# MycroftAI/mycroft-precise

Hardware: AMD Instinct MI355X
Metric: MFCC+GRU windows/sec (node); max concurrent real-time 16 kHz streams (higher is better)
Workload: dtype f32

## Files before the change

### include/precise_engine.h

```cpp
#ifndef PRECISE_ENGINE_H
#define PRECISE_ENGINE_H

#include <stddef.h>
#include <stdint.h>

#ifdef __cplusplus
extern "C" {
#endif

#define PE_ABI_VERSION 8

typedef enum pe_status {
    PE_OK = 0,
    PE_ERR_INVALID = 1,
    PE_ERR_HIP = 2,
    PE_ERR_UNSUPPORTED = 3,
    PE_ERR_NOMEM = 4,
    PE_ERR_EOF = 5
} pe_status;

typedef struct pe_params {
    int32_t sample_rate;
    int32_t window_samples;
    int32_t hop_samples;
// ... 65 lines not shown
                      float* feats_out_host);
int pe_update_vectors_device(pe_engine* e, const int16_t* pcm_dev, int32_t chunk_samples,
                             float* feats_out_dev, void* hip_stream);

int pe_get_vectors(pe_engine* e, float* feats_out_host);

int pe_set_vectors(pe_engine* e, const float* feats_host);

int pe_run_device(pe_engine* e, float* raw_out_dev, void* hip_stream);

int pe_predict(pe_engine* e, const float* feats_host, int32_t n, float* out_host);
int pe_predict_device(pe_engine* e, const float* feats_dev, int32_t n, float* out_dev,
                      void* hip_stream);

int pe_vectorize_raw(pe_engine* e, const double* audio_host, int64_t n_samples,
                     double* feats_out_host, int64_t max_frames, int64_t* n_frames_out);

int pe_vectorize_mels(pe_engine* e, const double* audio_host, int64_t n_samples,
                      double* mels_out_host, int64_t max_frames, int64_t* n_frames_out);

int pe_evaluate(pe_engine* e, const double* audio_host, int64_t n_samples, int32_t hop_frames,
                float* out_host, int64_t max_windows, int64_t* n_windows_out);

int pe_set_decoder(pe_engine* e, const double* cd, int32_t cd_len, int32_t min_out, int32_t out_range, double center);
int pe_set_trigger(pe_engine* e, int32_t chunk_size_bytes, double sensitivity, int32_t trigger_level);
int pe_set_decoder_model(pe_engine* e, int32_t model, const double* cd, int32_t cd_len, int32_t min_out, int32_t out_range, double center);
int pe_set_trigger_model(pe_engine* e, int32_t model, int32_t chunk_size_bytes, double sensitivity, int32_t trigger_level);
int pe_decode_device(pe_engine* e, const float* raw_dev, double* conf_out_dev, unsigned char* fired_out_dev, void* hip_stream);
int pe_decode(pe_engine* e, const float* raw_host, double* conf_out_host, unsigned char* fired_out_host);

typedef struct pe_info {
    int32_t n_streams, n_features, n_mfcc, units, n_layers, ring_slots, carry_capacity;
    int32_t mfcc_precision, gru_precision;
    int64_t device_bytes;
} pe_info;
int pe_get_info(const pe_engine* e, pe_info* out);

int pe_get_stream_state(pe_engine* e, int32_t* q_out, uint32_t* computed_out, uint32_t* emitted_out);

int pe_set_renumber_at(pe_engine* e, uint32_t call_number);

int pe_set_fused(pe_engine* e, int32_t enabled);

int pe_set_input_projection(pe_engine* e, int32_t enabled);

int pe_set_gru_waves(pe_engine* e, int32_t waves_per_tile);

int pe_set_gru_tiling(pe_engine* e, int32_t tiling);
int pe_get_gru_tiling(const pe_engine* e);

int pe_set_timing(pe_engine* e, int32_t enabled);
int pe_get_last_timing(pe_engine* e, float* mfcc_ms, float* gru_ms);

#ifdef __cplusplus
}
#endif
#endif
```

### mycroft_precise_amd/_lib.py

```python
import ctypes as C
import importlib.util
import os
import weakref

import numpy as np

HERE = os.path.dirname(os.path.abspath(__file__))
LIB_PATH = os.environ.get('PE_LIB') or os.path.join(HERE, 'libprecise_engine.so')

PE_OK, PE_ERR_INVALID, PE_ERR_HIP, PE_ERR_UNSUPPORTED, PE_ERR_NOMEM, PE_ERR_EOF = range(6)
ABI_VERSION = 8


class PeParams(C.Structure):
    _fields_ = [(n, C.c_int32) for n in (
        'sample_rate', 'window_samples', 'hop_samples', 'n_fft', 'n_filt', 'n_mfcc', 'n_features',
        'use_delta', 'mfcc_precision', 'gru_precision', 'vectorizer', 'ring_precision')]


class PeGruLayer(C.Structure):
    _fields_ = [('n_in', C.c_int32), ('units', C.c_int32),
                ('kernel', C.POINTER(C.c_float)), ('recurrent_kernel', C.POINTER(C.c_float)),
                ('bias', C.POINTER(C.c_float))]


class PeWeights(C.Structure):
    _fields_ = [('n_layers', C.c_int32), ('layers', C.POINTER(PeGruLayer)),
                ('dense_kernel', C.POINTER(C.c_float)), ('dense_bias', C.c_float)]


class PeInfo(C.Structure):
    _fields_ = [(n, C.c_int32) for n in (
        'n_streams', 'n_features', 'n_mfcc', 'units', 'n_layers', 'ring_slots', 'carry_capacity',
        'mfcc_precision', 'gru_precision')] + [('device_bytes', C.c_int64)]


EXPORTS = {
    'pe_abi_version': (C.c_int, []),
    'pe_last_global_error': (C.c_char_p, []),
    'pe_create': (C.c_int, [C.POINTER(PeParams), C.POINTER(C.c_double), C.POINTER(PeWeights), C.c_int32,
                            C.c_int32, C.POINTER(C.c_void_p)]),
    'pe_create_models': (C.c_int, [C.POINTER(PeParams), C.POINTER(C.c_double), C.POINTER(PeWeights), C.c_int32, C.c_int32,
                                   C.c_int32, C.POINTER(C.c_void_p)]),
    'pe_get_n_models': (C.c_int, [C.c_void_p]),
    'pe_destroy': (C.c_int, [C.c_void_p]),
    'pe_last_error': (C.c_char_p, [C.c_void_p]),
    'pe_clear': (C.c_int, [C.c_void_p, C.c_void_p]),
    'pe_update': (C.c_int, [C.c_void_p, C.c_void_p, C.c_int32, C.c_void_p]),
    'pe_update_device': (C.c_int, [C.c_void_p, C.c_void_p, C.c_int32, C.c_void_p, C.c_void_p]),
    'pe_update_device_keep': (C.c_int, [C.c_void_p, C.c_void_p, C.c_int32, C.c_void_p, C.c_void_p]),
    'pe_update_subset': (C.c_int, [C.c_void_p, C.c_void_p, C.c_int32, C.c_void_p, C.c_int32, C.c_void_p]),
    'pe_update_subset_device': (C.c_int, [C.c_void_p, C.c_void_p, C.c_int32, C.c_void_p, C.c_int32, C.c_void_p, C.c_void_p]),
    'pe_set_renumber_at': (C.c_int, [C.c_void_p, C.c_uint32]),
    'pe_host_alloc': (C.c_int, [C.c_void_p, C.c_size_t, C.POINTER(C.c_void_p)]),
    'pe_host_free': (C.c_int, [C.c_void_p, C.c_void_p]),
    'pe_update_async': (C.c_int, [C.c_void_p, C.c_void_p, C.c_int32, C.c_void_p]),
    'pe_wait': (C.c_int, [C.c_void_p]),
    'pe_reserve_updates': (C.c_int, [C.c_void_p, C.c_int32, C.c_int32]),
    'pe_update_many': (C.c_int, [C.c_void_p, C.c_void_p, C.c_int32, C.c_int32, C.c_void_p]),
    'pe_update_many_device': (C.c_int, [C.c_void_p, C.c_void_p, C.c_int32, C.c_int32, C.c_void_p, C.c_void_p]),
    'pe_update_vectors': (C.c_int, [C.c_void_p, C.c_void_p, C.c_int32, C.c_void_p]),
    'pe_update_vectors_device': (C.c_int, [C.c_void_p, C.c_void_p, C.c_int32, C.c_void_p, C.c_void_p]),
    'pe_get_vectors': (C.c_int, [C.c_void_p, C.c_void_p]),
    'pe_set_vectors': (C.c_int, [C.c_void_p, C.c_void_p]),
    'pe_run_device': (C.c_int, [C.c_void_p, C.c_void_p, C.c_void_p]),
    'pe_predict': (C.c_int, [C.c_void_p, C.c_void_p, C.c_int32, C.c_void_p]),
    'pe_predict_device': (C.c_int, [C.c_void_p, C.c_void_p, C.c_int32, C.c_void_p, C.c_void_p]),
# ... 391 lines not shown
```

### mycroft_precise_amd/csrc/engine.hip

```cpp
#include "../../include/precise_engine.h"
#include "pe_common.h"
#include "gru_cw_pack.h"
#include "mfcc_general_device.h"

#include <algorithm>
#include <cmath>
#include <cstdarg>
#include <cstdio>
#include <cstdlib>
#include <cstring>
#include <string>
#include <vector>

using namespace pe;

namespace {

thread_local std::string g_global_error;

struct DeviceBuf {
    void* p = nullptr;
    size_t bytes = 0;
};

// ... 1 lines not shown
    float dense_bias = 0.f;
    float* wxd = nullptr; float* wx = nullptr; float* wr1 = nullptr; float* wr2 = nullptr; float* bias = nullptr; float* wd = nullptr;
    float* cw_blob = nullptr;
    float* wide_buf[2][6] = {{nullptr}}; float* wide_wd = nullptr;
    float* wide3_buf[2][6] = {{nullptr}}; float* wide3_wd = nullptr;
    uint16_t* wx_bf16 = nullptr; uint16_t* wr_bf16 = nullptr; float* wd_bf16 = nullptr;
    uint32_t* b20_blob = nullptr;
    uint32_t* x3_blob = nullptr;
};
struct DecState {
    double* cd = nullptr; int cd_len = 0, min_out = 0, out_range = 0; double center = 0.5;
    double threshold = 0.5; int level = 3, rearm = -8; bool on = false;
};

}

struct pe_engine {
    pe_params prm{};
    int device = 0;
    int n_streams = 0, n_tiles = 0, n_padded = 0;
    int units = 0, n_in = 0, n_layers = 0;
    int ring_slots = 0;
    int mel_nnz = 0;
    std::string err;
    std::vector<void*> allocs;
    int64_t device_bytes = 0;
    StreamRec* rec = nullptr;
    int16_t* carry = nullptr;
    const int16_t* kept = nullptr; int kept_chunk = 0;
    const int16_t* call_head = nullptr; int call_head_chunk = 0; bool call_keep = false;
    uint32_t call_no = 1;
    uint32_t renumber_at = 0x7fff0000u;
    bool fused = true;
    int gru_waves = 0;
    bool general = false;
    int row_floats = kRowFloats;
    int carry_cap = kCarryCap;
    GeneralTables gtab{};
    int gru_tiling = -1;
    int n_cus = 256;
    float* ring = nullptr;
    float* proj_ring = nullptr;
    bool proj_ok = false, proj_on = false;
    std::vector<float> proj_w_host, proj_b_host;
    int max_updates = 1;
    uint32_t* ke_hist = nullptr;
    unsigned char* table_blob = nullptr;
    pe_wave::Layout table_layout{};
    int n_models = 1;
    std::vector<NetPack> nets;
    std::vector<DecState> dec;
    bool wide = false;
    int wide_kx4[2] = {1, 1};
    int32_t* activation = nullptr;
    DeviceBuf st_pcm, st_out, st_feats, st_mask, st_audio, st_mfcc, st_conf, st_fired, st_ids;
    std::vector<uint8_t> seen_ids;
    bool timing = false;
    hipEvent_t ev[3] = {nullptr, nullptr, nullptr};
    bool ev_valid = false, ev_has_gru = false;
    static constexpr int kAsyncDepth = 3;
    struct AsyncSlot {
        float* pin_out = nullptr; size_t pin_out_bytes = 0;
        DeviceBuf dev_in, dev_out;
        hipEvent_t copied = nullptr, done = nullptr;
        float* user_out = nullptr; size_t out_bytes = 0;
        bool direct_out = false, busy = false;
// ... 745 lines not shown
    e->user_dirty = true;
}

int check_chunk(pe_engine* e, const void* pcm, int chunk) {
    if (!e) return PE_ERR_INVALID;
    if (chunk == 0) return fail(e, PE_ERR_EOF, "empty chunk");
    if (chunk < 0 || !pcm) return fail(e, PE_ERR_INVALID, "bad pcm buffer / chunk_samples=%d", chunk);
    return PE_OK;
}

int flush_kept(pe_engine* e, hipStream_t s) {
    if (!e->kept) return PE_OK;
    PE_HIP(e, launch_materialize_carry(state_of(e, e->call_no + 1u), e->kept, e->kept_chunk, e->n_streams, s));
    e->kept = nullptr; e->kept_chunk = 0;
    return PE_OK;
}

bool keep_eligible(const pe_engine* e, const int16_t* pcm_dev, int chunk) {
    return !e->general && (chunk & 1) == 0 && (reinterpret_cast<uintptr_t>(pcm_dev) & 3u) == 0 && chunk >= frame_len_of(e->prm) - 1
        && chunk >= e->carry_cap - 1;
}

bool can_fuse(const pe_engine* e, int chunk) {
    if (!(e->fused && !e->general && !e->wide && e->table_layout.mel_pad == 10 && chunk <= emit_window(e->prm) - frame_len_of(e->prm))) return false;
    if (gru_args(e).x3) return false;
    if (e->prm.gru_precision == 0 && gru_small_regs(e->units) >= 6 && gru_args(e).waves_per_tile != 4) return false;
    if (e->prm.use_delta && e->prm.gru_precision == 0) {
        const GruArgs g = gru_args(e);
        if (g.cw && (g.waves_per_tile != 4 || e->ring_slots != kCwSlots || e->prm.n_features > kCwSlots)) return false;
    }
    return true;
}

int do_update(pe_engine* e, const int16_t* pcm_dev, int chunk, float* raw_out_dev, float* feats_out_dev,
              hipStream_t s, const int32_t* ids = nullptr, int n_active = 0, bool keep = false) {
    int rc;
    const bool t = e->timing;
    const bool keep_call = keep && !ids && keep_eligible(e, pcm_dev, chunk);
    if (keep_call && e->kept) {
        const char* a0 = reinterpret_cast<const char*>(e->kept);
        const char* a1 = a0 + (size_t)e->n_streams * e->kept_chunk * sizeof(int16_t);
        const char* b0 = reinterpret_cast<const char*>(pcm_dev);
        const char* b1 = b0 + (size_t)e->n_streams * chunk * sizeof(int16_t);
        if (b0 < a1 && a0 < b1)
            return fail(e, PE_ERR_INVALID, "pe_update_device_keep: this call's chunks overlap the previous call's (%p), which still hold the "
                        "streams' leftover samples -- alternate between at least two buffers, or use pe_update_device", (const void*)e->kept);
    }
    if (!keep_call && (rc = flush_kept(e, s))) return rc;
    e->call_head = keep_call ? e->kept : nullptr; e->call_head_chunk = e->kept_chunk; e->call_keep = keep_call;
    struct Reset { pe_engine* e; ~Reset() { e->call_head = nullptr; e->call_head_chunk = 0; e->call_keep = false; } } reset{e};
    e->kept = keep_call ? pcm_dev : nullptr; e->kept_chunk = keep_call ? chunk : 0;
    uint32_t call = 0;
    if ((rc = begin_state_call(e, s, &call))) return rc;
    if (t) { PE_HIP(e, hipEventRecord(e->ev[0], s)); }
    if (raw_out_dev && can_fuse(e, chunk)) {
        GruArgs g = gru_args(e);
        g.call = call;
        g.predict_ke = 1;
        g.chunk = chunk;
        g.out = raw_out_dev;
        if (ids) { g.ids = ids; g.n_streams = n_active; }
        const ModelSet ms = model_set(e, g);
        const ModelSet* const models = e->n_models > 1 ? &ms : nullptr;
        if (e->prm.mfcc_precision == 0) PE_HIP(e, launch_fused(mfcc_args<double>(e, pcm_dev, chunk, call, ids, n_active), tables<double>(e), g, e->n_cus, s, models, e->n_models));
        else PE_HIP(e, launch_fused(mfcc_args<float>(e, pcm_dev, chunk, call, ids, n_active), tables<float>(e), g, e->n_cus, s, models, e->n_models));
        if (t) { PE_HIP(e, hipEventRecord(e->ev[1], s)); PE_HIP(e, hipEventRecord(e->ev[2], s)); e->ev_valid = true; e->ev_has_gru = false; }
    } else {
        if ((rc = launch_mfcc(e, pcm_dev, chunk, s, call, ids, n_active))) return rc;
        if (t) { PE_HIP(e, hipEventRecord(e->ev[1], s)); }
        if (raw_out_dev) {
            if ((rc = launch_gru_ring(e, raw_out_dev, s, ids, n_active))) return rc;
        }
        if (t) { PE_HIP(e, hipEventRecord(e->ev[2], s)); e->ev_valid = true; e->ev_has_gru = raw_out_dev != nullptr; }
    }
    if (feats_out_dev) {
        GatherArgs g{e->n_streams, e->prm.n_features, e->prm.n_mfcc, e->ring_slots, e->prm.ring_precision, e->ring, state_of(e, e->call_no + 1u), feats_out_dev, e->row_floats};
        PE_HIP(e, launch_gather(g, s));
    }
    return PE_OK;
}

}

extern "C" {

int pe_abi_version(void) { return PE_ABI_VERSION; }
const char* pe_last_global_error(void) { return g_global_error.c_str(); }
const char* pe_last_error(const pe_engine* e) { return e ? e->err.c_str() : g_global_error.c_str(); }

namespace {
int create_engine(const pe_params* p, const double* mel_filters, const pe_weights* w, int32_t n_models, int32_t n_streams,
                  int32_t device, pe_engine** out) {
    if (!p || !mel_filters || !w || !out) return fail(nullptr, PE_ERR_INVALID, "null argument to pe_create");
    *out = nullptr;
    if (n_streams <= 0) return fail(nullptr, PE_ERR_INVALID, "n_streams must be positive, got %d", n_streams);
    if (p->n_fft < 16 || p->n_fft > kGeneralMaxFft || (!general_is_pow2(p->n_fft) && p->n_fft > kGeneralMaxBlueFft))
        return fail(nullptr, PE_ERR_UNSUPPORTED, "n_fft must be any length in 16..%d or a power of two up to %d (got %d)", kGeneralMaxBlueFft, kGeneralMaxFft, p->n_fft);
    if (p->n_mfcc < 1 || p->n_mfcc > kGeneralMaxMfcc) return fail(nullptr, PE_ERR_UNSUPPORTED, "n_mfcc must be in 1..%d (got %d)", kGeneralMaxMfcc, p->n_mfcc);
// ... 771 lines not shown
        }
        return PE_OK;
    }
    g.waves_per_tile = 1;
    return launch_networks_many(e, g, n_updates, s);
}

int pe_update_many(pe_engine* e, const int16_t* pcm_host, int32_t chunk, int32_t n_updates, float* raw_out_host) {
    int rc = check_chunk(e, pcm_host, chunk);
    if (rc) return rc;
    if (!raw_out_host || n_updates < 1) return fail(e, PE_ERR_INVALID, "bad arguments to pe_update_many");
    PE_HIP(e, hipSetDevice(e->device));
    const size_t pcm_bytes = (size_t)n_updates * e->n_streams * chunk * sizeof(int16_t);
    const size_t out_bytes = (size_t)e->n_models * n_updates * e->n_streams * sizeof(float);
    if ((rc = ensure(e, e->st_pcm, pcm_bytes))) return rc;
    if ((rc = ensure(e, e->st_out, out_bytes))) return rc;
    PE_HIP(e, hipMemcpy(e->st_pcm.p, pcm_host, pcm_bytes, hipMemcpyHostToDevice));
    if ((rc = pe_update_many_device(e, static_cast<const int16_t*>(e->st_pcm.p), chunk, n_updates, static_cast<float*>(e->st_out.p), nullptr))) return rc;
    PE_HIP(e, hipMemcpy(raw_out_host, e->st_out.p, out_bytes, hipMemcpyDeviceToHost));
    return PE_OK;
}

int pe_get_info(const pe_engine* e, pe_info* out) {
    if (!e || !out) return PE_ERR_INVALID;
    out->n_streams = e->n_streams;
    out->n_features = e->prm.n_features;
    out->n_mfcc = e->prm.n_mfcc;
    out->units = e->units;
    out->n_layers = e->n_layers;
    out->ring_slots = e->ring_slots;
    out->carry_capacity = e->carry_cap;
    out->mfcc_precision = e->prm.mfcc_precision;
    out->gru_precision = e->prm.gru_precision;
    out->device_bytes = e->device_bytes;
    return PE_OK;
}

int pe_get_stream_state(pe_engine* e, int32_t* q_out, uint32_t* computed_out, uint32_t* emitted_out) {
    if (!e) return PE_ERR_INVALID;
    PE_HIP(e, hipSetDevice(e->device));
    PE_DRAIN(e);
    PE_HIP(e, hipDeviceSynchronize());
    std::vector<StreamRec> host((size_t)2 * e->n_padded);
    PE_HIP(e, hipMemcpy(host.data(), e->rec, host.size() * sizeof(StreamRec), hipMemcpyDeviceToHost));
    const uint32_t call = e->call_no + 1u;
    for (int s = 0; s < e->n_streams; ++s) {
        const StreamRec& r0 = host[rec_at((uint32_t)e->n_padded, s, 0)];
        const StreamRec& r1 = host[rec_at((uint32_t)e->n_padded, s, 1)];
        const StreamRec& c = (call - r1.wcall) - 1u < (call - r0.wcall) - 1u ? r1 : r0;
        if (q_out) q_out[s] = c.q;
        if (computed_out) computed_out[s] = c.kc;
        if (emitted_out) emitted_out[s] = c.ke;
    }
    return PE_OK;
}

int pe_set_renumber_at(pe_engine* e, uint32_t call_number) {
    if (!e) return PE_ERR_INVALID;
    if (call_number < 8u || call_number > 0x7fff0000u) return fail(e, PE_ERR_INVALID, "renumbering threshold must be in 8..0x7fff0000");
    e->renumber_at = call_number;
    return PE_OK;
}

int pe_set_fused(pe_engine* e, int32_t enabled) {
    if (!e) return PE_ERR_INVALID;
    PE_DRAIN(e);
// ... 76 lines not shown
```

### mycroft_precise_amd/csrc/kernels.hip

```cpp
#include <cstdlib>
#include <type_traits>
#include "mfcc_device.h"
#include "mfcc_wave_device.h"
#include "gru_device.h"
#include "gru_cw_device.h"
#include "gru_bf16_device.h"
#include "gru_b20_device.h"
#include "gru_x3_device.h"
#include "gru_wide_device.h"
#include "gru_wide_x3_device.h"
#include "mfcc_general_device.h"

namespace pe {

#ifndef PE_FRAME_WPE
#define PE_FRAME_WPE 4
#endif
template <int BYTES>
__device__ __forceinline__ void touch_kernel_arguments() {
    const int* ka = (const int*)__builtin_amdgcn_kernarg_segment_ptr();
    static_assert(BYTES <= 12 * 64, "more lines than this helper requests");
    auto line = [&](int i) -> int { return i * 64 < BYTES ? ka[i * 16] : 0; };
    const int v0 = line(0), v1 = line(1), v2 = line(2), v3 = line(3), v4 = line(4), v5 = line(5), v6 = line(6), v7 = line(7),
              v8 = line(8), v9 = line(9), v10 = line(10), v11 = line(11);
    asm volatile("" :: "s"(v0), "s"(v1), "s"(v2), "s"(v3), "s"(v4), "s"(v5), "s"(v6), "s"(v7), "s"(v8), "s"(v9), "s"(v10), "s"(v11));
}

#if defined(__HIP_DEVICE_COMPILE__)
#define PE_NO_PK_F32 __attribute__((target("no-packed-fp32-ops")))
#else
#define PE_NO_PK_F32
#endif
#define PE_UNPAREN(...) __VA_ARGS__
#define PE_KERNEL_PAIR(TEMPLATE, ATTRS, NAME, PARAMS, ...)                                                   \
    PE_UNPAREN TEMPLATE __global__ PE_UNPAREN ATTRS void NAME PARAMS __VA_ARGS__                            \
    PE_UNPAREN TEMPLATE __global__ PE_UNPAREN ATTRS PE_NO_PK_F32 void NAME##_nopk PARAMS __VA_ARGS__
#define PE_FRAME_KERNEL(THREADS, WPE) (__launch_bounds__(THREADS) __attribute__((amdgpu_waves_per_eu(WPE))))
#define PE_LAUNCH_R(R, KERNEL, TARGS, ...)                                                                   \
// ... 303 lines not shown
                    __syncthreads();
                    if (((1 << slot[0]) | (1 << slot[1]) | (1 << slot[2]) | (1 << slot[3])) == 15) role = simd;
                }
                gru_tile_cw<false>(gm, bl, role, threadIdx.x & 63, reinterpret_cast<float*>(smem));
            } else {
                const int tile = bl * 4 + wave;
                if (tile < n_tiles) gru_tile_v<kRing, false>(gm, tile, threadIdx.x & 63);
            }
        } else if (MW) {
            gru_tile_mw_any<RG, PROJ>(gm, bl, wave, threadIdx.x & 63, reinterpret_cast<float*>(smem));
        } else {
            const int tile = bl * 4 + wave;
            if (tile < n_tiles) gru_tile<RG, kRing, PROJ>(gm, tile, threadIdx.x & 63);
        }
    } else if (b < n_net + n_frame_blocks) {
        mfcc_frame_tasks<R, SH, true, !PROJ>(m, t, smem, (b - n_net) * kFrameWaves, n_frame_blocks * kFrameWaves, CW && MW && (frames_first & kBySimd));
    } else {
        mfcc_book_tile<R>(m, b - n_net - n_frame_blocks);
    }
}

#define PE_FUSED_PARAMS (const MfccStreamArgs<R> m, const WaveTables<R> t, const GruArgs g, const int n_gru_blocks, const int n_frame_blocks, const int n_tiles, const int frames_first)
#define PE_FUSED_MODELS_PARAMS (const MfccStreamArgs<R> m, const WaveTables<R> t, const GruArgs g, const int n_gru_blocks, const int n_models, const int n_frame_blocks, \
                                const int n_tiles, const int frames_first, const ModelSet ms)
PE_KERNEL_PAIR((template <class R, class SH, bool DELTA, bool RB>), PE_FRAME_KERNEL(256, PE_FRAME_WPE), fused_update_bf16_kernel, PE_FUSED_PARAMS,
               { fused_update_bf16_body<R, SH, DELTA, RB, false>(m, t, g, nullptr, n_gru_blocks, 1, n_frame_blocks, n_tiles, frames_first); })
PE_KERNEL_PAIR((template <class R, class SH, bool DELTA, bool RB>), PE_FRAME_KERNEL(256, PE_FRAME_WPE), fused_update_bf16_models_kernel, PE_FUSED_MODELS_PARAMS,
               { fused_update_bf16_body<R, SH, DELTA, RB, true>(m, t, g, &ms, n_gru_blocks, n_models, n_frame_blocks, n_tiles, frames_first); })
PE_KERNEL_PAIR((template <class R, class SH, int RG, bool MW, bool PROJ, bool CW = false>), PE_FRAME_KERNEL(256, PE_FRAME_WPE), fused_update_kernel, PE_FUSED_PARAMS,
               { fused_update_body<R, SH, RG, MW, PROJ, CW, false>(m, t, g, nullptr, n_gru_blocks, 1, n_frame_blocks, n_tiles, frames_first); })
PE_KERNEL_PAIR((template <class R, class SH, int RG, bool MW, bool CW>), PE_FRAME_KERNEL(256, PE_FRAME_WPE), fused_update_models_kernel, PE_FUSED_MODELS_PARAMS,
               { fused_update_body<R, SH, RG, MW, false, CW, true>(m, t, g, &ms, n_gru_blocks, n_models, n_frame_blocks, n_tiles, frames_first); })


static int frame_blocks(long long n_tasks, int n_cus, int per_cu = 4) {
    const long long need = (n_tasks + kFrameWaves - 1) / kFrameWaves;
    const long long cap = (long long)n_cus * per_cu;
    return (int)(need < cap ? (need < 1 ? 1 : need) : cap);
}

static int stream_frame_blocks(int n_streams, int n_cus, int per_cu_default = 4) {
    const long long slots = 2LL * n_streams;
    const long long cap_waves = (long long)frame_blocks(slots, n_cus, per_cu_default) * kFrameWaves;
    const long long per_wave = (slots + cap_waves - 1) / cap_waves;
    const long long waves = (slots + per_wave - 1) / per_wave;
    return (int)((waves + kFrameWaves - 1) / kFrameWaves);
}

template <class R>
static size_t frame_lds(const WaveTables<R>& t) { return wave_lds_bytes(sizeof(R), t.L, kFrameWaves); }
template <class R>
static bool blob_matches_shape(const WaveTables<R>& t) {
    return t.L.mel_pad == ShapeStock::MEL ? shape_layout_matches<R, ShapeStock>(t.L) : shape_layout_matches<R, ShapeAny>(t.L);
}

template <class R>
static hipError_t launch_mfcc(const MfccStreamArgs<R>& a, const WaveTables<R>& t, int n_cus, hipStream_t s) {
    const int tiles = (a.geo.n_streams + kTileStreams - 1) / kTileStreams;
    const int fb = stream_frame_blocks(a.geo.n_streams, n_cus);
    if (!blob_matches_shape(t)) return hipErrorInvalidValue;
    const bool single = a.n_updates == 1 && !a.proj_ring;
    if (t.L.mel_pad == ShapeStock::MEL) {
        if (single) PE_LAUNCH_R(R, mfcc_kernel, (ShapeStock, true), dim3(fb + tiles), dim3(64 * kFrameWaves), frame_lds(t), s, a, t, fb);
        else PE_LAUNCH_R(R, mfcc_kernel, (ShapeStock), dim3(fb + tiles), dim3(64 * kFrameWaves), frame_lds(t), s, a, t, fb);
    } else {
        if (single) PE_LAUNCH_R(R, mfcc_kernel, (ShapeAny, true), dim3(fb + tiles), dim3(64 * kFrameWaves), frame_lds(t), s, a, t, fb);
// ... 153 lines not shown
    else return hipErrorInvalidValue;
    return hipGetLastError();
}

template <class R>
static hipError_t launch_fused_t(const MfccStreamArgs<R>& m, const WaveTables<R>& t, const GruArgs& g, int n_cus, hipStream_t s,
                                 const ModelSet* ms, int n_models) {
    if (ms && (n_models < 1 || n_models > kMaxModels)) return hipErrorInvalidValue;
    if (t.L.mel_pad != ShapeStock::MEL || !blob_matches_shape(t)) return hipErrorInvalidValue;
    if (g.bf16) {
        const int tiles = (m.geo.n_streams + kTileStreams - 1) / kTileStreams;
        const int tpw = 4;
        const int gru_blocks = (tiles + tpw - 1) / tpw;
        const int ff = tiles >= 4 * n_cus ? 1 : 0;
        const int frames_first = (ff & 1) | (tpw << 8);
        const FusedLaunch f{ms, n_models, stream_frame_blocks(m.geo.n_streams, n_cus, ff ? 3 : 4), tiles, s};
        with_flag(g.use_delta, [&](auto D) { with_flag(g.ring_bf16, [&](auto RB) {
            PE_FUSED(fused_update_bf16_kernel, fused_update_bf16_models_kernel, (ShapeStock, PE_CONST(D), PE_CONST(RB)), (ShapeStock, PE_CONST(D), PE_CONST(RB)),
                     gru_blocks, frame_lds(t), frames_first); }); });
        return hipGetLastError();
    }
    hipError_t err = hipErrorInvalidValue;
    with_const<1, 2, 3, 4, 5, 6, 7, 8>(gru_small_regs(g.units), [&](auto RG) { err = launch_fused_rg<R, PE_CONST(RG)>(m, t, g, n_cus, s, ms, n_models); });
    return err;
}

hipError_t launch_fused(const MfccStreamArgs<double>& m, const WaveTables<double>& t, const GruArgs& g, int n_cus, hipStream_t s, const ModelSet* ms, int n_models) {
    return launch_fused_t<double>(m, t, g, n_cus, s, ms, n_models);
}
hipError_t launch_fused(const MfccStreamArgs<float>& m, const WaveTables<float>& t, const GruArgs& g, int n_cus, hipStream_t s, const ModelSet* ms, int n_models) {
    return launch_fused_t<float>(m, t, g, n_cus, s, ms, n_models);
}

#ifndef PE_GEN_TWO_WAVES
#define PE_GEN_TWO_WAVES 0
#endif
template <class R, int BITS, bool BLUE = false>
__global__ __launch_bounds__(64) __attribute__((amdgpu_waves_per_eu(BITS >= 10 ? 2 : 4))) void mfcc_general_stream_kernel(const GeneralStreamArgs<R> a) {
    extern __shared__ __attribute__((aligned(16))) unsigned char smem[];
    const int s = PE_GEN_TWO_WAVES ? blockIdx.x >> 1 : blockIdx.x;
    if (s < a.geo.n_streams) general_stream<R, BITS, BLUE>(a, reinterpret_cast<R*>(smem), s, PE_GEN_TWO_WAVES ? blockIdx.x & 1 : 0, threadIdx.x, PE_GEN_TWO_WAVES ? 2 : 1);
}
template <class R, int BITS, bool BLUE = false>
__global__ __launch_bounds__(64) __attribute__((amdgpu_waves_per_eu(BITS >= 10 ? 2 : 4))) PE_NO_PK_F32 void mfcc_general_stream_kernel_nopk(const GeneralStreamArgs<R> a) {
    extern __shared__ __attribute__((aligned(16))) unsigned char smem[];
    const int s = PE_GEN_TWO_WAVES ? blockIdx.x >> 1 : blockIdx.x;
    if (s < a.geo.n_streams) general_stream<R, BITS, BLUE>(a, reinterpret_cast<R*>(smem), s, PE_GEN_TWO_WAVES ? blockIdx.x & 1 : 0, threadIdx.x, PE_GEN_TWO_WAVES ? 2 : 1);
}
template <class R, int BITS, bool BLUE = false>
__global__ __launch_bounds__(64) __attribute__((amdgpu_waves_per_eu(BITS >= 10 ? 2 : 4))) void mfcc_general_offline_kernel(const GeneralOfflineArgs<R> a) {
    extern __shared__ __attribute__((aligned(16))) unsigned char smem[];
    general_offline<R, BITS, BLUE>(a, reinterpret_cast<R*>(smem), blockIdx.x, gridDim.x, threadIdx.x);
}
template <class R, int BITS, bool BLUE = false>
__global__ __launch_bounds__(64) __attribute__((amdgpu_waves_per_eu(BITS >= 10 ? 2 : 4))) PE_NO_PK_F32 void mfcc_general_offline_kernel_nopk(const GeneralOfflineArgs<R> a) {
    extern __shared__ __attribute__((aligned(16))) unsigned char smem[];
    general_offline<R, BITS, BLUE>(a, reinterpret_cast<R*>(smem), blockIdx.x, gridDim.x, threadIdx.x);
}
template <class F>
static bool with_general_bits(const GeneralTables& tab, F&& f) {
    if (tab.chirp) return with_const<7, 8, 9, 10, 11>(tab.log2m, [&](auto B) { f(B, std::true_type{}); });
    return with_const<5, 6, 7, 8, 9, 10>(tab.log2m, [&](auto B) { f(B, std::false_type{}); });
}
template <class R>
static hipError_t launch_general_stream_t(const GeneralStreamArgs<R>& a, hipStream_t s) {
    if (a.geo.n_streams == 0) return hipSuccess;
// ... 213 lines not shown
```

### mycroft_precise_amd/csrc/pe_common.h

```cpp
#pragma once
#include <hip/hip_runtime.h>
#include <stdint.h>
#include "mfcc_wave_tables.h"

namespace pe {

constexpr int kTileStreams = 16;
constexpr int kRowFloats = 16;
constexpr int kCarryCap = 512;
constexpr int kNfft = 512;
constexpr int kBins = kNfft / 2 + 1;
constexpr int kMaxFilt = 64;
constexpr int kCwSlots = 32;

template <class R> struct cplx { R x, y; };

constexpr int kMaxFrameRows = 4096;
constexpr int kFrameWaves = 4;

template <class R>
struct WaveTables {
    const void* blob;
    pe_wave::Layout L;
};
// ... 93 lines not shown
constexpr int kX3Tiles = 4;
constexpr int kX3RecOps = 4, kX3InOps = 3;
constexpr int kX3ArOff = 0;
constexpr int kX3AxOff = kX3Tiles * kX3RecOps * 64;
constexpr int kX3WdOff = kX3AxOff + kX3Tiles * kX3InOps * 64;
constexpr int kX3BlobBytes = kX3WdOff * 16 + 5 * 64 * 4;

constexpr int kB20Tiles = 4;
constexpr int kB20ArOff = 0;
constexpr int kB20AxOff = kB20Tiles * 64;
constexpr int kB20WdOff = 2 * kB20Tiles * 64;
constexpr int kB20BlobBytes = kB20WdOff * 16 + 5 * 64 * 4;

struct GruArgs {
    int n_streams;
    int n_features;
    int n_in;
    int units;
    const float* wx;
    const float* wxd;
    int use_delta;
    const float* wr1;
    const float* wr2;
    const float* bias;
    const float* wd;
    float dense_bias;
    const float* cw;
    int bf16;
    const void* wx_bf16;
    const void* wr_bf16;
    const float* wd_bf16;
    const void* b20;
    const void* x3;
    const void* reserved_;
    const int32_t* ids;
    const StreamRec* rec;
    uint32_t n_padded, call;
    const uint32_t* ke_plain;
    const float* ring;
    int ring_bf16;
    const float* proj_ring;
    int ring_slots;
    int predict_ke;
    int chunk, window, hop, frame_len;
    const float* feats;
    int row_stride;
    float* out;
    int row_floats;
    int waves_per_tile;
};

constexpr int kMaxModels = 8;
struct ModelNet {
    const float* wx; const float* wxd; const float* wr1; const float* wr2; const float* bias; const float* wd;
    const float* cw;
    const void* wx_bf16; const void* wr_bf16; const float* wd_bf16; const void* b20;
    const void* x3;
    float dense_bias;
};
struct ModelSet { ModelNet net[kMaxModels]; };
__host__ __device__ __forceinline__ GruArgs model_args(const GruArgs& a, const ModelNet& n, const int m, const long long out_stride) {
    GruArgs b = a;
    b.wx = n.wx; b.wxd = n.wxd; b.wr1 = n.wr1; b.wr2 = n.wr2; b.bias = n.bias; b.wd = n.wd;
    b.cw = n.cw;
    b.wx_bf16 = n.wx_bf16; b.wr_bf16 = n.wr_bf16; b.wd_bf16 = n.wd_bf16; b.b20 = n.b20;
    b.x3 = n.x3;
    b.dense_bias = n.dense_bias;
// ... 61 lines not shown
    const uint8_t* mask;
    StreamState st;
    float* ring;
    int ring_bf16;
    int32_t* activation;
    float* proj_ring;
    const float* proj_b;
    int row_floats = kRowFloats;
};

struct DecodeArgs {
    int n_streams;
    const float* raw;
    const double* cd;
    int cd_len, min_out, out_range;
    double center;
    double* conf_out;
    int32_t* activation;
    unsigned char* fired_out;
    double threshold;
    int trigger_level, rearm;
};
hipError_t launch_decode(const DecodeArgs& a, hipStream_t s);
struct DecodeSet { DecodeArgs m[kMaxModels]; };
hipError_t launch_decode_models(const DecodeSet& d, int n_models, int n_streams, hipStream_t s);
hipError_t launch_clear_activation(const uint8_t* mask, int32_t* activation, int n_streams, int n_padded, int n_rows, hipStream_t s);

constexpr int kProjRow = pe_wave::kProjRow;
hipError_t launch_mfcc_f64(const MfccStreamArgs<double>& a, const WaveTables<double>& t, int n_cus, hipStream_t s);
hipError_t launch_mfcc_f32(const MfccStreamArgs<float>& a, const WaveTables<float>& t, int n_cus, hipStream_t s);
hipError_t launch_gru_many(const GruArgs& a, int n_updates, int n_padded, hipStream_t s, const ModelSet* ms = nullptr, int n_models = 1);
hipError_t launch_fused(const MfccStreamArgs<double>& m, const WaveTables<double>& t, const GruArgs& g, int n_cus, hipStream_t s, const ModelSet* ms = nullptr, int n_models = 1);
hipError_t launch_fused(const MfccStreamArgs<float>& m, const WaveTables<float>& t, const GruArgs& g, int n_cus, hipStream_t s, const ModelSet* ms = nullptr, int n_models = 1);
hipError_t launch_mfcc_offline_f64(const MfccOfflineArgs<double>& a, const WaveTables<double>& t, int n_cus, hipStream_t s);
hipError_t launch_mfcc_offline_f32(const MfccOfflineArgs<float>& a, const WaveTables<float>& t, int n_cus, hipStream_t s);
hipError_t launch_gru_small(const GruArgs& a, int input_mode, hipStream_t s, const ModelSet* ms = nullptr, int n_models = 1, long long out_stride = 0);
int gru_small_regs(int units);
int gru_wide_waves(int units);
int gru_small_tiles(int units);
hipError_t launch_gru_wide(const WideArgs& a, int input_mode, hipStream_t s);
hipError_t launch_gru_wide_x3(const WideArgs& a, int input_mode, hipStream_t s);
hipError_t launch_gather(const GatherArgs& a, hipStream_t s);
hipError_t launch_scatter(const GatherArgs& a, hipStream_t s);
hipError_t launch_renumber(const StreamState& st, int n_padded, hipStream_t s);
hipError_t launch_materialize_carry(const StreamState& st, const int16_t* head, int head_chunk, int n_streams, hipStream_t s);
hipError_t launch_clear(const ClearArgs& a, hipStream_t s);
hipError_t launch_project_rows(const float* ring, float* proj, const float* w, const float* b, int n_mfcc, long long n_rows, hipStream_t s);

}
```

Before: 271.8 million.

## Carry per-slot GRU hidden chains across calls instead of recomputing full windows

Adds a persistent device buffer holding one GRU hidden state per ring slot, with one chain per possible window start. A new fused kernel advances every live chain by the one or two newly computed frames and emits the finished window's state to the dense head. This replaces replaying the full window's serial recurrence on each update. A rebuild kernel reconstructs the chains from the ring whenever they are stale, such as on first use or when calls were skipped. The cost is extra device memory, a state-validity path that depends on call numbering, and a narrow eligibility gate: single model, f32 GRU, cw layout, no delta features, small chunks.

```diff
diff --git a/include/precise_engine.h b/include/precise_engine.h
--- a/include/precise_engine.h
+++ b/include/precise_engine.h
@@ -121,6 +121,7 @@
 typedef struct pe_info {
     int32_t n_streams, n_features, n_mfcc, units, n_layers, ring_slots, carry_capacity;
     int32_t mfcc_precision, gru_precision;
+    int32_t chain_carry;
     int64_t device_bytes;
 } pe_info;
 int pe_get_info(const pe_engine* e, pe_info* out);
diff --git a/mycroft_precise_amd/_lib.py b/mycroft_precise_amd/_lib.py
--- a/mycroft_precise_amd/_lib.py
+++ b/mycroft_precise_amd/_lib.py
@@ -32,7 +32,7 @@
 class PeInfo(C.Structure):
     _fields_ = [(n, C.c_int32) for n in (
         'n_streams', 'n_features', 'n_mfcc', 'units', 'n_layers', 'ring_slots', 'carry_capacity',
-        'mfcc_precision', 'gru_precision')] + [('device_bytes', C.c_int64)]
+        'mfcc_precision', 'gru_precision', 'chain_carry')] + [('device_bytes', C.c_int64)]
 
 
 EXPORTS = {
diff --git a/mycroft_precise_amd/csrc/engine.hip b/mycroft_precise_amd/csrc/engine.hip
--- a/mycroft_precise_amd/csrc/engine.hip
+++ b/mycroft_precise_amd/csrc/engine.hip
@@ -57,6 +57,9 @@
     uint32_t call_no = 1;
     uint32_t renumber_at = 0x7fff0000u;
     bool fused = true;
+    float* chains = nullptr;
+    uint32_t chain_call = 0;
+    int chain_carry = 0;
     int gru_waves = 0;
     bool general = false;
     int row_floats = kRowFloats;
@@ -868,6 +871,12 @@
     return true;
 }
 
+bool chain_eligible(const pe_engine* e, const GruArgs& g, int chunk) {
+    const int hop = e->prm.hop_samples;
+    return e->n_models == 1 && e->prm.gru_precision == 0 && chain_shape_ok(g) && e->n_tiles <= 2 * e->n_cus
+        && (chunk + hop - 1) / hop <= chain_max_frames();
+}
+
 int do_update(pe_engine* e, const int16_t* pcm_dev, int chunk, float* raw_out_dev, float* feats_out_dev,
               hipStream_t s, const int32_t* ids = nullptr, int n_active = 0, bool keep = false) {
     int rc;
@@ -887,19 +896,39 @@
     struct Reset { pe_engine* e; ~Reset() { e->call_head = nullptr; e->call_head_chunk = 0; e->call_keep = false; } } reset{e};
     e->kept = keep_call ? pcm_dev : nullptr; e->kept_chunk = keep_call ? chunk : 0;
     uint32_t call = 0;
+    const bool chains_valid = e->chains && e->chain_call == e->call_no;
+    e->chain_carry = 0;
     if ((rc = begin_state_call(e, s, &call))) return rc;
     if (t) { PE_HIP(e, hipEventRecord(e->ev[0], s)); }
     if (raw_out_dev && can_fuse(e, chunk)) {
         GruArgs g = gru_args(e);
         g.call = call;
-        g.predict_ke = 1;
-        g.chunk = chunk;
-        g.out = raw_out_dev;
-        if (ids) { g.ids = ids; g.n_streams = n_active; }
-        const ModelSet ms = model_set(e, g);
-        const ModelSet* const models = e->n_models > 1 ? &ms : nullptr;
-        if (e->prm.mfcc_precision == 0) PE_HIP(e, launch_fused(mfcc_args<double>(e, pcm_dev, chunk, call, ids, n_active), tables<double>(e), g, e->n_cus, s, models, e->n_models));
-        else PE_HIP(e, launch_fused(mfcc_args<float>(e, pcm_dev, chunk, call, ids, n_active), tables<float>(e), g, e->n_cus, s, models, e->n_models));
+        if (chain_eligible(e, g, chunk)) {
+            if (!e->chains) {
+                const size_t floats = (size_t)e->n_tiles * kCwSlots * 5 * 64;
+                if ((rc = dev_alloc(e, &e->chains, floats))) return rc;
+                PE_HIP(e, hipMemsetAsync(e->chains, 0, floats * sizeof(float), s));
+            }
+            g.chains = e->chains;
+            if (!chains_valid) PE_HIP(e, launch_chain_rebuild(g, s));
+            g.predict_ke = 1;
+            g.chunk = chunk;
+            g.out = raw_out_dev;
+            if (ids) { g.ids = ids; g.n_streams = n_active; }
+            if (e->prm.mfcc_precision == 0) PE_HIP(e, launch_fused_chain(mfcc_args<double>(e, pcm_dev, chunk, call, ids, n_active), tables<double>(e), g, e->n_cus, s));
+            else PE_HIP(e, launch_fused_chain(mfcc_args<float>(e, pcm_dev, chunk, call, ids, n_active), tables<float>(e), g, e->n_cus, s));
+            e->chain_call = call;
+            e->chain_carry = chains_valid ? 1 : 2;
+        } else {
+            g.predict_ke = 1;
+            g.chunk = chunk;
+            g.out = raw_out_dev;
+            if (ids) { g.ids = ids; g.n_streams = n_active; }
+            const ModelSet ms = model_set(e, g);
+            const ModelSet* const models = e->n_models > 1 ? &ms : nullptr;
+            if (e->prm.mfcc_precision == 0) PE_HIP(e, launch_fused(mfcc_args<double>(e, pcm_dev, chunk, call, ids, n_active), tables<double>(e), g, e->n_cus, s, models, e->n_models));
+            else PE_HIP(e, launch_fused(mfcc_args<float>(e, pcm_dev, chunk, call, ids, n_active), tables<float>(e), g, e->n_cus, s, models, e->n_models));
+        }
         if (t) { PE_HIP(e, hipEventRecord(e->ev[1], s)); PE_HIP(e, hipEventRecord(e->ev[2], s)); e->ev_valid = true; e->ev_has_gru = false; }
     } else {
         if ((rc = launch_mfcc(e, pcm_dev, chunk, s, call, ids, n_active))) return rc;
@@ -1737,6 +1766,7 @@
     out->carry_capacity = e->carry_cap;
     out->mfcc_precision = e->prm.mfcc_precision;
     out->gru_precision = e->prm.gru_precision;
+    out->chain_carry = e->chain_carry;
     out->device_bytes = e->device_bytes;
     return PE_OK;
 }
diff --git a/mycroft_precise_amd/csrc/gru_chain_device.h b/mycroft_precise_amd/csrc/gru_chain_device.h
--- /dev/null
+++ b/mycroft_precise_amd/csrc/gru_chain_device.h
@@ -0,0 +1,170 @@
+#pragma once
+#include "gru_cw_device.h"
+
+namespace pe {
+
+constexpr int kChainNmax = 2;
+constexpr int kChainTileFloats = kCwSlots * 5 * 64;
+constexpr int kChainLdsFloats = kChainNmax * 4 * 256;
+constexpr size_t kChainLdsBytes = (size_t)kChainLdsFloats * sizeof(float);
+
+__device__ __forceinline__ float* chain_base(float* chains, const long long sid, const int g) {
+    return chains + (size_t)(sid >> 4) * kChainTileFloats + g * 16 + (int)(sid & 15);
+}
+
+__device__ __forceinline__ void gru_chain_advance(const GruArgs& a, const int tile, const int wave, const int lane, float* S) {
+#pragma clang fp contract(off)
+    const int g = lane >> 4, j = lane & 15;
+    const long long stream = (long long)tile * kTileStreams + j;
+    const bool valid = stream < a.n_streams;
+    const uint32_t T = (uint32_t)a.n_features;
+    const float* cw = a.cw;
+    const long long sid = gru_stream_of(a, stream, valid);
+    const KeRequest req = gru_ke_request(a, sid);
+    const float* const xbase = a.ring + gru_ring_cell(a, sid) * kRowFloats + 4 * g;
+    float* const hbase = chain_base(a.chains, sid, g);
+    CwStep<false> St;
+    St.load(cw, lane);
+    float wx[4], bb[4], wd[5];
+#pragma unroll
+    for (int kk = 0; kk < 4; ++kk) {
+        wx[kk] = cw[CwPack::WX + (wave * 4 + kk) * 64 + lane];
+        bb[kk] = cw[CwPack::BIAS + (wave * 4 + kk) * 64 + lane];
+    }
+#pragma unroll
+    for (int rho = 0; rho < 5; ++rho) wd[rho] = a.wd[rho * 64 + lane];
+    const uint32_t ke0 = rec_pick(req.p, rec_side(req.p, a.call)).ke;
+    const uint32_t ke1 = gru_ke_resolve(a, req);
+    const uint32_t n = ke1 - ke0;
+    int nw = 0;
+#pragma unroll
+    for (int i = 0; i < kChainNmax; ++i)
+        if (__builtin_amdgcn_ballot_w64(n > (uint32_t)i) != 0) nw = i + 1;
+    const f32x4 bias = {bb[0], bb[1], bb[2], bb[3]};
+#pragma unroll
+    for (int i = 0; i < kChainNmax; ++i) {
+        const uint32_t slot = (ke0 + (uint32_t)i) & (uint32_t)(kCwSlots - 1);
+        const f32x4 x = *reinterpret_cast<const f32x4*>(xbase + (size_t)slot * kTileStreams * kRowFloats);
+        *reinterpret_cast<f32x4*>(S + ((i * 4 + wave) * 64 + lane) * 4) = cw_xproj(wx, bias, x);
+    }
+    St.pin();
+    cw_barrier();
+    const uint32_t out_slot = (ke1 - T) & 31u;
+    float hout[5];
+#pragma unroll
+    for (int rho = 0; rho < 5; ++rho) hout[rho] = 0.f;
+    auto load_h = [&](const uint32_t c, float (&h)[5]) {
+#pragma unroll
+        for (int rho = 0; rho < 5; ++rho) h[rho] = hbase[(c * 5 + rho) * 64];
+    };
+    auto advance = [&](float (&h)[5], const uint32_t c, const uint32_t e, const bool has, bool& dirty,
+                       const f32x4& aZ, const f32x4& aX, const f32x4& aC, const f32x4& aV) {
+        const bool fresh = c == (e & 31u);
+        float hn[5];
+#pragma unroll
+        for (int rho = 0; rho < 5; ++rho) hn[rho] = fresh ? 0.f : h[rho];
+        St.step(hn, aZ, aX, aC, aV);
+        const bool live = has && ((e - c) & 31u) < T;
+#pragma unroll
+        for (int rho = 0; rho < 5; ++rho) h[rho] = live ? hn[rho] : h[rho];
+        dirty = dirty || live;
+    };
+    auto finish = [&](const float (&h)[5], const uint32_t c, const bool dirty) {
+#pragma unroll
+        for (int rho = 0; rho < 5; ++rho) {
+            if (c == out_slot) hout[rho] = h[rho];
+            if (valid && dirty) hbase[(c * 5 + rho) * 64] = h[rho];
+        }
+    };
+    float hA[5], hB[5];
+    load_h((uint32_t)wave * 8u, hA);
+    load_h((uint32_t)wave * 8u + 1u, hB);
+#pragma unroll 1
+    for (int b = 0; b < 4; ++b) {
+        const uint32_t cA = (uint32_t)wave * 8u + 2u * (uint32_t)b, cB = cA + 1u;
+        float nA[5], nB[5];
+        const uint32_t cN = b < 3 ? cA + 2u : cA;
+        load_h(cN, nA);
+        load_h(cN + 1u, nB);
+        bool dA = false, dB = false;
+        for (int i = 0; i < nw; ++i) {
+            const f32x4 aZ = *reinterpret_cast<const f32x4*>(S + ((i * 4 + kTZ) * 64 + lane) * 4);
+            const f32x4 aX = *reinterpret_cast<const f32x4*>(S + ((i * 4 + kTX) * 64 + lane) * 4);
+            const f32x4 aC = *reinterpret_cast<const f32x4*>(S + ((i * 4 + kTC) * 64 + lane) * 4);
+            const f32x4 aV = *reinterpret_cast<const f32x4*>(S + ((i * 4 + kTV) * 64 + lane) * 4);
+            const uint32_t e = ke0 + (uint32_t)i;
+            const bool has = (uint32_t)i < n;
+            advance(hA, cA, e, has, dA, aZ, aX, aC, aV);
+            advance(hB, cB, e, has, dB, aZ, aX, aC, aV);
+        }
+        finish(hA, cA, dA);
+        finish(hB, cB, dB);
+#pragma unroll
+        for (int rho = 0; rho < 5; ++rho) { hA[rho] = nA[rho]; hB[rho] = nB[rho]; }
+    }
+    cw_head(a, hout, wd, stream, valid && (int)(out_slot >> 3) == wave, g);
+}
+
+__device__ __forceinline__ void gru_chain_rebuild(const GruArgs& a, const int tile, const int wave, const int lane) {
+#pragma clang fp contract(off)
+    const int g = lane >> 4, j = lane & 15;
+    const long long sid = (long long)tile * kTileStreams + j;
+    const bool valid = sid < a.n_streams;
+    const uint32_t T = (uint32_t)a.n_features;
+    const float* cw = a.cw;
+    const uint32_t ke = gru_window_end(a, sid);
+    const float* const xbase = a.ring + gru_ring_cell(a, sid) * kRowFloats + 4 * g;
+    float* const hbase = chain_base(a.chains, sid, g);
+    CwStep<false> St;
+    St.load(cw, lane);
+    float wx[4][4];
+    f32x4 bias[4];
+#pragma unroll
+    for (int tl = 0; tl < 4; ++tl)
+#pragma unroll
+        for (int kk = 0; kk < 4; ++kk) {
+            wx[tl][kk] = cw[CwPack::WX + (tl * 4 + kk) * 64 + lane];
+            bias[tl][kk] = cw[CwPack::BIAS + (tl * 4 + kk) * 64 + lane];
+        }
+#pragma unroll 1
+    for (int p = 0; p < 4; ++p) {
+        const int k = p == 0 ? wave : p == 1 ? 7 - wave : p == 2 ? 8 + wave : 15 - wave;
+        const uint32_t cA = 2u * (uint32_t)k, cB = cA + 1u;
+        uint32_t lenA = ((ke - 1u - cA) & 31u) + 1u, lenB = ((ke - 1u - cB) & 31u) + 1u;
+        if (lenA > T) lenA = 0u;
+        if (lenB > T) lenB = 0u;
+        int lmax = (int)(lenA > lenB ? lenA : lenB);
+#pragma unroll
+        for (int d = 1; d < 64; d <<= 1) { const int o = __shfl_xor(lmax, d); lmax = o > lmax ? o : lmax; }
+        const uint32_t L = (uint32_t)__builtin_amdgcn_readfirstlane(lmax);
+        float hA[5], hB[5];
+#pragma unroll
+        for (int rho = 0; rho < 5; ++rho) hA[rho] = hB[rho] = 0.f;
+        auto row = [&](const uint32_t t) -> f32x4 {
+            const uint32_t slot = (ke - L + t) & (uint32_t)(kCwSlots - 1);
+            return *reinterpret_cast<const f32x4*>(xbase + (size_t)slot * kTileStreams * kRowFloats);
+        };
+        f32x4 x = row(0u);
+        for (uint32_t t = 0; t < L; ++t) {
+            const f32x4 xn = row(t + 1u < L ? t + 1u : t);
+            const f32x4 aZ = cw_xproj(wx[kTZ], bias[kTZ], x), aX = cw_xproj(wx[kTX], bias[kTX], x);
+            const f32x4 aC = cw_xproj(wx[kTC], bias[kTC], x), aV = cw_xproj(wx[kTV], bias[kTV], x);
+            float nA[5], nB[5];
+#pragma unroll
+            for (int rho = 0; rho < 5; ++rho) { nA[rho] = hA[rho]; nB[rho] = hB[rho]; }
+            St.step(nA, aZ, aX, aC, aV);
+            St.step(nB, aZ, aX, aC, aV);
+            const bool onA = t + lenA >= L, onB = t + lenB >= L;
+#pragma unroll
+            for (int rho = 0; rho < 5; ++rho) { hA[rho] = onA ? nA[rho] : hA[rho]; hB[rho] = onB ? nB[rho] : hB[rho]; }
+            x = xn;
+        }
+#pragma unroll
+        for (int rho = 0; rho < 5; ++rho) {
+            if (valid && lenA != 0u) hbase[(cA * 5 + rho) * 64] = hA[rho];
+            if (valid && lenB != 0u) hbase[(cB * 5 + rho) * 64] = hB[rho];
+        }
+    }
+}
+
+}
diff --git a/mycroft_precise_amd/csrc/kernels.hip b/mycroft_precise_amd/csrc/kernels.hip
--- a/mycroft_precise_amd/csrc/kernels.hip
+++ b/mycroft_precise_amd/csrc/kernels.hip
@@ -4,6 +4,7 @@
 #include "mfcc_wave_device.h"
 #include "gru_device.h"
 #include "gru_cw_device.h"
+#include "gru_chain_device.h"
 #include "gru_bf16_device.h"
 #include "gru_b20_device.h"
 #include "gru_x3_device.h"
@@ -373,6 +374,35 @@
 PE_KERNEL_PAIR((template <class R, class SH, int RG, bool MW, bool CW>), PE_FRAME_KERNEL(256, PE_FRAME_WPE), fused_update_models_kernel, PE_FUSED_MODELS_PARAMS,
                { fused_update_body<R, SH, RG, MW, false, CW, true>(m, t, g, &ms, n_gru_blocks, n_models, n_frame_blocks, n_tiles, frames_first); })
 
+#ifndef PE_CHAIN_PRIO
+#define PE_CHAIN_PRIO 3
+#endif
+#ifndef PE_CHAIN_BY_SIMD
+#define PE_CHAIN_BY_SIMD 0
+#endif
+template <class R, class SH>
+__device__ __forceinline__ void fused_update_chain_body(const MfccStreamArgs<R>& m, const WaveTables<R>& t, const GruArgs& g,
+                                                        const int n_gru_blocks, const int n_frame_blocks) {
+    extern __shared__ __attribute__((aligned(16))) unsigned char smem[];
+    touch_kernel_arguments<kFusedArgBytes<R, false>>();
+    const int b = blockIdx.x;
+    if (b < n_gru_blocks) {
+        const int wave = __builtin_amdgcn_readfirstlane(threadIdx.x >> 6);
+        __builtin_amdgcn_s_setprio(PE_CHAIN_PRIO);
+        gru_chain_advance(g, b, wave, threadIdx.x & 63, reinterpret_cast<float*>(smem));
+    } else if (b < n_gru_blocks + n_frame_blocks) {
+        mfcc_frame_tasks<R, SH, true, true>(m, t, smem, (b - n_gru_blocks) * kFrameWaves, n_frame_blocks * kFrameWaves, PE_CHAIN_BY_SIMD != 0);
+    } else {
+        mfcc_book_tile<R>(m, b - n_gru_blocks - n_frame_blocks);
+    }
+}
+PE_KERNEL_PAIR((template <class R, class SH>), PE_FRAME_KERNEL(256, PE_FRAME_WPE), fused_update_chain_kernel, PE_FUSED_PARAMS,
+               { (void)n_tiles; (void)frames_first; fused_update_chain_body<R, SH>(m, t, g, n_gru_blocks, n_frame_blocks); })
+__global__ __launch_bounds__(256) void gru_chain_rebuild_kernel(const GruArgs a) {
+    touch_kernel_arguments<(int)sizeof(GruArgs)>();
+    gru_chain_rebuild(a, blockIdx.x, __builtin_amdgcn_readfirstlane(threadIdx.x >> 6), threadIdx.x & 63);
+}
+
 
 static int frame_blocks(long long n_tasks, int n_cus, int per_cu = 4) {
     const long long need = (n_tasks + kFrameWaves - 1) / kFrameWaves;
@@ -592,6 +622,34 @@
     return launch_fused_t<float>(m, t, g, n_cus, s, ms, n_models);
 }
 
+int chain_max_frames() { return kChainNmax; }
+bool chain_shape_ok(const GruArgs& g) {
+    return g.cw && !g.bf16 && !g.x3 && !g.use_delta && !g.proj_ring && g.row_floats == kRowFloats && g.waves_per_tile == 4 && cw_four_waves_ok(g)
+        && g.n_features + kChainNmax <= kCwSlots;
+}
+template <class R>
+static hipError_t launch_fused_chain_t(const MfccStreamArgs<R>& m, const WaveTables<R>& t, const GruArgs& g, int n_cus, hipStream_t s) {
+    if (t.L.mel_pad != ShapeStock::MEL || !blob_matches_shape(t) || !chain_shape_ok(g) || !g.chains || !g.predict_ke) return hipErrorInvalidValue;
+    const int tiles = (m.geo.n_streams + kTileStreams - 1) / kTileStreams;
+    const int fb = stream_frame_blocks(m.geo.n_streams, n_cus, tiles <= n_cus ? 2 : 4);
+    const size_t lds = frame_lds(t) > kChainLdsBytes ? frame_lds(t) : kChainLdsBytes;
+    PE_LAUNCH_R(R, fused_update_chain_kernel, (ShapeStock), dim3(tiles + fb + tiles), dim3(256), lds, s, m, t, g, tiles, fb, tiles, 0);
+    return hipGetLastError();
+}
+hipError_t launch_fused_chain(const MfccStreamArgs<double>& m, const WaveTables<double>& t, const GruArgs& g, int n_cus, hipStream_t s) {
+    return launch_fused_chain_t<double>(m, t, g, n_cus, s);
+}
+hipError_t launch_fused_chain(const MfccStreamArgs<float>& m, const WaveTables<float>& t, const GruArgs& g, int n_cus, hipStream_t s) {
+    return launch_fused_chain_t<float>(m, t, g, n_cus, s);
+}
+hipError_t launch_chain_rebuild(const GruArgs& g, hipStream_t s) {
+    if (!chain_shape_ok(g) || !g.chains || g.ids || g.predict_ke || g.ke_plain) return hipErrorInvalidValue;
+    const int tiles = (g.n_streams + kTileStreams - 1) / kTileStreams;
+    if (tiles == 0) return hipSuccess;
+    hipLaunchKernelGGL(gru_chain_rebuild_kernel, dim3(tiles), dim3(256), 0, s, g);
+    return hipGetLastError();
+}
+
 #ifndef PE_GEN_TWO_WAVES
 #define PE_GEN_TWO_WAVES 0
 #endif
diff --git a/mycroft_precise_amd/csrc/pe_common.h b/mycroft_precise_amd/csrc/pe_common.h
--- a/mycroft_precise_amd/csrc/pe_common.h
+++ b/mycroft_precise_amd/csrc/pe_common.h
@@ -149,7 +149,7 @@
     const float* wd_bf16;
     const void* b20;
     const void* x3;
-    const void* reserved_;
+    float* chains;
     const int32_t* ids;
     const StreamRec* rec;
     uint32_t n_padded, call;
@@ -277,6 +277,11 @@
 hipError_t launch_gru_many(const GruArgs& a, int n_updates, int n_padded, hipStream_t s, const ModelSet* ms = nullptr, int n_models = 1);
 hipError_t launch_fused(const MfccStreamArgs<double>& m, const WaveTables<double>& t, const GruArgs& g, int n_cus, hipStream_t s, const ModelSet* ms = nullptr, int n_models = 1);
 hipError_t launch_fused(const MfccStreamArgs<float>& m, const WaveTables<float>& t, const GruArgs& g, int n_cus, hipStream_t s, const ModelSet* ms = nullptr, int n_models = 1);
+int chain_max_frames();
+bool chain_shape_ok(const GruArgs& g);
+hipError_t launch_fused_chain(const MfccStreamArgs<double>& m, const WaveTables<double>& t, const GruArgs& g, int n_cus, hipStream_t s);
+hipError_t launch_fused_chain(const MfccStreamArgs<float>& m, const WaveTables<float>& t, const GruArgs& g, int n_cus, hipStream_t s);
+hipError_t launch_chain_rebuild(const GruArgs& g, hipStream_t s);
 hipError_t launch_mfcc_offline_f64(const MfccOfflineArgs<double>& a, const WaveTables<double>& t, int n_cus, hipStream_t s);
 hipError_t launch_mfcc_offline_f32(const MfccOfflineArgs<float>& a, const WaveTables<float>& t, int n_cus, hipStream_t s);
 hipError_t launch_gru_small(const GruArgs& a, int input_mode, hipStream_t s, const ModelSet* ms = nullptr, int n_models = 1, long long out_stride = 0);
```

Measured after the change: 269.3 million. No clear change (-0.9%).
